# thethomasboyer/PhenDiff

Hardware: AMD Instinct MI355X
Metric: img2img images/sec (50-step DDIM invert+denoise, 256x256) (higher is better)
Workload: dtype bf16; 1 GPU; configs[2]: 256x256 pipeline_conditional_ddim invert->class-swap->denoise, 50+50 DDIM steps, super_small UNet (random init, seed 0), 3k_steps_clipping_rescaling, 32 images/GPU/step sharded over 1 GPU(s), no collectives; batch_per_gpu=32, global_batch=32, inference_steps=50, image_size=256, hipgraph=True, concurrent_trajectories=1

## Files before the change

phendiff_amd/csrc/attn_d8.hip:

```cpp
#include <stdlib.h>
#include <type_traits>
#include "pd_common.h"

namespace pd {

constexpr int KT = 256;
static_assert(KT == 256, "knmax is read as one f32x4 (KT / 64 slices)");

typedef uint32_t u32x4 __attribute__((ext_vector_type(4)));

__device__ __forceinline__ float row16_max(float x) {
#define PD_DPP_MAX(ctrl) x = fmaxf(x, __int_as_float(__builtin_amdgcn_update_dpp(__float_as_int(x), __float_as_int(x), ctrl, 0xf, 0xf, false)))
  PD_DPP_MAX(0xB1);
  PD_DPP_MAX(0x4E);
  PD_DPP_MAX(0x141);
  PD_DPP_MAX(0x140);
#undef PD_DPP_MAX
  return x;
}

__device__ __forceinline__ unsigned short bits16(bf16_t v) { return v; }
__device__ __forceinline__ unsigned short bits16(half_t v) { return v.bits; }

template <typename T> struct AttnOps {
  static constexpr float RESCALE_THR = sizeof(T) == 2 && !std::is_same<T, bf16_t>::value ? 14.0f : 16.0f;
  static constexpr int VT_PITCH = (KT + 8) * 2;
  struct QF { s16x8 v; };
  static __device__ __forceinline__ QF load_q(const T* q, int h, float scale) {
    QF f; f.v = (s16x8)(0);
    if (h == 0) {
      s16x8 raw = *(const s16x8*)q;
      {
        float x[8];
        typename Elem<T>::Frag fr; fr.v = raw;
        Elem<T>::unpack(fr, x);
#pragma unroll
        for (int j = 0; j < 8; ++j) x[j] *= scale;
        f.v = Elem<T>::pack(x).v;
      }
    }
    return f;
  }
  static constexpr float M_C0 = std::is_same<T, bf16_t>::value ? 1.0f : 4096.0f;
  static constexpr bool M_IN_C = false;
  static __device__ __forceinline__ float set_m(QF& q, f32x16&, int h, float m) {
    const T hi = Elem<T>::from_f(-m * (1.0f / M_C0));
    const float r1 = fmaf(-M_C0, Elem<T>::to_f(hi), -m);
    const T mid = Elem<T>::from_f(r1);
    const float r2 = r1 - Elem<T>::to_f(mid);
    const T lo = Elem<T>::from_f(r2);
    if (h) { q.v[0] = (short)bits16(hi); q.v[1] = (short)bits16(mid); q.v[2] = (short)bits16(lo); }
    return -(fmaf(M_C0, Elem<T>::to_f(hi), Elem<T>::to_f(mid)) + Elem<T>::to_f(lo));
  }
  static __device__ __forceinline__ void split3(float x, T& hi, T& mid, T& lo) {
    hi = Elem<T>::from_f(x * (1.0f / M_C0));
    const float r1 = fmaf(-M_C0, Elem<T>::to_f(hi), x);
    mid = Elem<T>::from_f(r1);
    lo = Elem<T>::from_f(r1 - Elem<T>::to_f(mid));
  }
  static __device__ __forceinline__ void set_terms(QF& q, int h, float c) {
    T hi, mid, lo;
    split3(c, hi, mid, lo);
    if (h) { q.v[0] = (short)bits16(hi); q.v[1] = (short)bits16(mid); q.v[2] = (short)bits16(lo); }
  }
  static __device__ __forceinline__ void set_ones(QF& q, int h) {
    if (h) { q.v[0] = (short)bits16(Elem<T>::from_f(M_C0)); q.v[1] = (short)bits16(Elem<T>::from_f(1.0f)); q.v[2] = q.v[1]; }
  }
  static __device__ __forceinline__ void store_terms(unsigned char* row16, float c) {
    T t[8];
    split3(c, t[0], t[1], t[2]);
#pragma unroll
    for (int i = 3; i < 8; ++i) t[i] = Elem<T>::from_f(0.0f);
    *(s16x8*)row16 = *(const s16x8*)t;
  }
  static __device__ __forceinline__ void init_const_slot(unsigned char* slot) {
    T c[8];
#pragma unroll
    for (int i = 0; i < 8; ++i) c[i] = Elem<T>::from_f(i == 0 ? M_C0 : i < 3 ? 1.0f : 0.0f);
    *(s16x8*)slot = *(const s16x8*)c;
  }
  static __device__ __forceinline__ float q_norm2(const QF& q) {
    float x[8], t = 0.f;
    typename Elem<T>::Frag fr; fr.v = q.v;
    Elem<T>::unpack(fr, x);
#pragma unroll
    for (int j = 0; j < 8; ++j) t += x[j] * x[j];
    return t;
  }
  static __device__ __forceinline__ float dot(const QF& x, const QF& y) {
    float a[8], b[8], t = 0.f;
    typename Elem<T>::Frag fa, fb; fa.v = x.v; fb.v = y.v;
    Elem<T>::unpack(fa, a); Elem<T>::unpack(fb, b);
#pragma unroll
    for (int j = 0; j < 8; ++j) t += a[j] * b[j];
    return t;
  }
  static __device__ __forceinline__ float k_norm2(const typename Elem<T>::Frag& k) {
    const u32x4 w = __builtin_bit_cast(u32x4, k.v);
    float n2 = 0.f;
    if constexpr (std::is_same<T, bf16_t>::value) {
      typedef __bf16 bf2 __attribute__((ext_vector_type(2)));
#pragma unroll
      for (int j = 0; j < 4; ++j) {
        const uint32_t wj = w[j];
        const bf2 pr = __builtin_bit_cast(bf2, wj);
        n2 = __builtin_amdgcn_fdot2_f32_bf16(pr, pr, n2, false);
      }
    } else {
      float x[8];
      Elem<T>::unpack(k, x);
#pragma unroll
      for (int j = 0; j < 8; ++j) n2 += x[j] * x[j];
    }
    return n2;
  }
  static __device__ __forceinline__ void store_vt(unsigned char* vl, int vp, const typename Elem<T>::Frag& v) {
#pragma unroll
    for (int d = 0; d < 8; ++d) *(unsigned short*)(vl + d * VT_PITCH + vp * 2) = (unsigned short)v.v[d];
  }
  static constexpr int KROW = 16;
  static constexpr int KSTEP = 32 * KROW;
  static __device__ __forceinline__ int kaddr(int r, int h) { return h ? KT * KROW : r * KROW; }
  static __device__ __forceinline__ int kstep(int h) { return h ? 0 : KSTEP; }
  struct KF { s16x8 v; };
  struct VF { u32x4 v[2]; };
  static __device__ __forceinline__ KF load_k(const unsigned char* ka) { KF f; f.v = *(const s16x8*)ka; return f; }
  static __device__ __forceinline__ f32x16 qk(const KF& a, const QF& q, const f32x16& c) {
    return Elem<T>::mma16(a.v, q.v, c);
  }
  static __device__ __forceinline__ VF load_v(const unsigned char* vrow, int key0) {
    VF f;
    f.v[0] = *(const u32x4*)(vrow + key0 * 2);
    f.v[1] = *(const u32x4*)(vrow + (key0 + 16) * 2);
    return f;
  }
  static __device__ __forceinline__ int vpos(int t) { return t ^ ((((t >> 2) ^ (t >> 3)) & 1) * 12); }
  static __device__ __forceinline__ int vlane_off(int h) { return h * 16; }
  static __device__ __forceinline__ uint32_t pack_p(float lo, float hi) {
    if constexpr (std::is_same<T, bf16_t>::value) return __builtin_amdgcn_perm(__float_as_uint(hi), __float_as_uint(lo), 0x07060302u);
    else return Pack16<T>::pack(lo, hi);
  }
  static __device__ __forceinline__ f32x16 pv(const VF& a, const f32x16& p, f32x16 o) {
#pragma unroll
    for (int s = 0; s < 2; ++s) {
      uint32_t bw[4];
#pragma unroll
      for (int j = 0; j < 4; ++j) bw[j] = pack_p(p[8 * s + 2 * j], p[8 * s + 2 * j + 1]);
      u32x4 bv = {bw[0], bw[1], bw[2], bw[3]};
      o = Elem<T>::mma16(__builtin_bit_cast(s16x8, a.v[s]), __builtin_bit_cast(s16x8, bv), o);
    }
    return o;
  }
};

template <> struct AttnOps<float> {
  static constexpr float RESCALE_THR = 16.0f;
  static constexpr int VT_PITCH = (KT + 4) * 4;
  struct QF { f32x4 v; };
  static __device__ __forceinline__ QF load_q(const float* q, int h, float scale) {
    QF f; f.v = *(const f32x4*)(q + 4 * h);
    f.v *= scale;
    return f;
  }
  static constexpr bool M_IN_C = true;
  static __device__ __forceinline__ float set_m(QF&, f32x16& negm, int, float m) { negm = (f32x16)(-m); return m; }
  static __device__ __forceinline__ void init_const_slot(unsigned char*) {}
  static __device__ __forceinline__ float q_norm2(const QF& q) {
    return q.v[0] * q.v[0] + q.v[1] * q.v[1] + q.v[2] * q.v[2] + q.v[3] * q.v[3];
  }
  static __device__ __forceinline__ float dot(const QF& x, const QF& y) {
    return x.v[0] * y.v[0] + x.v[1] * y.v[1] + x.v[2] * y.v[2] + x.v[3] * y.v[3];
  }
  static __device__ __forceinline__ float k_norm2(const Elem<float>::Frag& k) {
    float n2 = 0.f;
#pragma unroll
    for (int j = 0; j < 4; ++j) n2 += k.lo[j] * k.lo[j] + k.hi[j] * k.hi[j];
    return n2;
  }
  static __device__ __forceinline__ void store_vt(unsigned char* vl, int vp, const Elem<float>::Frag& v) {
#pragma unroll
    for (int d = 0; d < 4; ++d) { *(float*)(vl + d * VT_PITCH + vp * 4) = v.lo[d]; *(float*)(vl + (4 + d) * VT_PITCH + vp * 4) = v.hi[d]; }
  }
  static constexpr int KROW = 32;
  static constexpr int KSTEP = 32 * KROW;
  static __device__ __forceinline__ int kaddr(int r, int h) { return r * KROW + h * 16; }
  static __device__ __forceinline__ int kstep(int) { return KSTEP; }
  static __device__ __forceinline__ int vpos(int t) { return t; }
  static __device__ __forceinline__ int vlane_off(int h) { return h * 16; }
  struct KF { f32x4 v; };
  struct VF { f32x4 v[4]; };
  static __device__ __forceinline__ KF load_k(const unsigned char* ka) { KF f; f.v = *(const f32x4*)ka; return f; }
  static __device__ __forceinline__ f32x16 qk(const KF& a, const QF& q, f32x16 c) {
#pragma unroll
    for (int i = 0; i < 4; ++i) c = __builtin_amdgcn_mfma_f32_32x32x2f32(a.v[i], q.v[i], c, 0, 0, 0);
    return c;
  }
  static __device__ __forceinline__ VF load_v(const unsigned char* vrow, int key0) {
    VF f;
#pragma unroll
    for (int g = 0; g < 4; ++g) f.v[g] = *(const f32x4*)(vrow + (key0 + 8 * g) * 4);
    return f;
  }
  static __device__ __forceinline__ f32x16 pv(const VF& a, const f32x16& p, f32x16 o) {
#pragma unroll
    for (int g = 0; g < 4; ++g)
#pragma unroll
      for (int i = 0; i < 4; ++i) o = __builtin_amdgcn_mfma_f32_32x32x2f32(a.v[g][i], p[4 * g + i], o, 0, 0, 0);
    return o;
  }
};

template <typename T, int QB, int WPB>
__global__ __launch_bounds__(WPB * 64) void attn_kernel(const pd_attn_args a) {
  constexpr int QPW = 32 * QB;
  constexpr int QPB = WPB * QPW;
  using E = Elem<T>;
  using Ops = AttnOps<T>;
  constexpr bool PIPE = sizeof(T) == 2 && QB == 1;
  constexpr int KROW = Ops::KROW;
  constexpr int VBYTES = 10 * Ops::VT_PITCH;
  __shared__ __attribute__((aligned(16))) unsigned char klds[2][KT * KROW + 16];
  __shared__ __attribute__((aligned(16))) unsigned char vlds[2][VBYTES];
  __shared__ __attribute__((aligned(16))) float knmax[2][KT / 64];

  const int tid = threadIdx.x, lane = tid & 63, wave = tid >> 6;
  const int r = lane & 31, h = lane >> 5;
  const int nqb = (a.N + QPB - 1) / QPB;
  const int total = nqb * a.heads * a.B;
  int item = blockIdx.x;
  if ((total & 7) == 0) item = (blockIdx.x & 7) * (total >> 3) + (blockIdx.x >> 3);
  const int qb = item % nqb;
  const int head = (item / nqb) % a.heads, b = item / (nqb * a.heads);
  const int N = a.N;
  const size_t bh = ((size_t)b * a.heads + head) * N;
  const T* qp = (const T*)a.q + bh * 8;
  const T* kp = (const T*)a.k + bh * 8;
  const T* vp = (const T*)a.v + bh * 8;

  const float qscale = 0.35355339059327373f * 1.4426950408889634f;
  constexpr float RESCALE_THR = Ops::RESCALE_THR;
  int query[QB];
  typename Ops::QF qf[QB];
  f32x16 o[QB], negm[QB];
  float qn[QB], m[QB];
  bool first[QB];
#pragma unroll
  for (int j = 0; j < QB; ++j) {
    query[j] = qb * QPB + (wave * QB + j) * 32 + r;
    qf[j] = Ops::load_q(qp + (size_t)min(query[j], N - 1) * 8, h, qscale);
    float t = Ops::q_norm2(qf[j]);
    t += __shfl_xor(t, 32);
    qn[j] = sqrtf(t) * 1.00001f + 1e-6f;
    o[j] = (f32x16)(0.f); negm[j] = (f32x16)(0.f); m[j] = 0.f; first[j] = true;
  }

#pragma unroll
  for (int b2 = 0; b2 < 2; ++b2) {
    if (tid == 0) { *(f32x4*)(klds[b2] + KT * KROW) = (f32x4)(0.f); Ops::init_const_slot(klds[b2] + KT * KROW); }
    if (tid < KT) { *(T*)(vlds[b2] + 8 * Ops::VT_PITCH + tid * E::BYTES) = E::from_f(1.0f); *(T*)(vlds[b2] + 9 * Ops::VT_PITCH + tid * E::BYTES) = E::from_f(0.0f); }
  }
  const int vrow_off = (r < 8 ? r : (r == 8 || r == 12) ? 8 : 9) * Ops::VT_PITCH + Ops::vlane_off(h);
  const int ka0 = Ops::kaddr(r, h), kst = Ops::kstep(h);

  const int st = tid & (KT - 1);
  const int my_parity = (WPB * 64 > KT) ? (tid / KT) : 0;
  auto mine = [&](int tile) { return (WPB * 64 > KT) ? ((tile & 1) == my_parity) : true; };
  typename E::Frag stk, stv;
  auto issue = [&](int k0) {
    if (!mine(k0 / KT)) return;
    const int key = k0 + st;
    if (key < N) { stk = E::load(kp + (size_t)key * 8); stv = E::load(vp + (size_t)key * 8); }
    else { stk = E::zero(); stv = E::zero(); }
  };
  auto commit = [&](int b2, int k0) {
    if (!mine(k0 / KT)) return;
    E::store(klds[b2] + st * KROW, stk);
    float n2 = row16_max(Ops::k_norm2(stk));
    n2 = fmaxf(n2, __shfl_xor(n2, 16));
    n2 = fmaxf(n2, __shfl_xor(n2, 32));
    if ((st & 63) == 0) knmax[b2][st >> 6] = sqrtf(n2) * 1.00002f;
    Ops::store_vt(vlds[b2], Ops::vpos(st), stv);
  };

  issue(0);
  commit(0, 0);
  if (KT < N) issue(KT);
  __syncthreads();
  for (int k0 = 0, cur = 0; k0 < N; k0 += KT, cur ^= 1) {
    const unsigned char* kl = klds[cur];
    const unsigned char* vrow = vlds[cur] + vrow_off;
    const f32x4 kn4 = *(const f32x4*)knmax[cur];
    const float kn8 = fmaxf(fmaxf(kn4[0], kn4[1]), fmaxf(kn4[2], kn4[3]));
    const bool full_tile = k0 + KT <= N;
    bool need = false;
#pragma unroll
    for (int j = 0; j < QB; ++j) need = need || first[j] || (qn[j] * kn8 - m[j] > RESCALE_THR);
    if (full_tile && !__builtin_amdgcn_ballot_w64(need)) {
      if constexpr (PIPE) {
        typename Ops::KF kfn = Ops::load_k(kl + ka0);
        typename Ops::VF vfn = Ops::load_v(vrow, 0);
        f32x16 sn = Ops::qk(kfn, qf[0], negm[0]);
        kfn = Ops::load_k(kl + ka0 + kst);
#pragma unroll
        for (int sub = 0; sub < KT / 32; ++sub) {
          const typename Ops::VF vf = vfn;
          f32x16 s = sn;
          if (sub + 1 < KT / 32) {
            sn = Ops::qk(kfn, qf[0], negm[0]);
            if (sub + 2 < KT / 32) kfn = Ops::load_k(kl + ka0 + (sub + 2) * kst);
            vfn = Ops::load_v(vrow, (sub + 1) * 32);
            __builtin_amdgcn_sched_barrier(0);
          }
#pragma unroll
          for (int i = 0; i < 16; ++i) s[i] = __builtin_amdgcn_exp2f(s[i]);
          o[0] = Ops::pv(vf, s, o[0]);
        }
      } else {
#pragma unroll
        for (int sub = 0; sub < KT / 32; ++sub) {
          const typename Ops::KF kf = Ops::load_k(kl + ka0 + sub * kst);
          const typename Ops::VF vf = Ops::load_v(vrow, sub * 32);
          f32x16 s[QB];
#pragma unroll
          for (int j = 0; j < QB; ++j) s[j] = Ops::qk(kf, qf[j], negm[j]);
#pragma unroll
          for (int j = 0; j < QB; ++j) {
#pragma unroll
            for (int i = 0; i < 16; ++i) s[j][i] = __builtin_amdgcn_exp2f(s[j][i]);
            o[j] = Ops::pv(vf, s[j], o[j]);
          }
        }
      }
    } else {
#pragma unroll 1
      for (int sub = 0; sub < KT / 32; ++sub) {
        const int kb = sub * 32;
        if (k0 + kb >= N) break;
        const typename Ops::KF kf = Ops::load_k(kl + ka0 + sub * kst);
        const typename Ops::VF vf = Ops::load_v(vrow, kb);
#pragma unroll
        for (int j = 0; j < QB; ++j) {
          f32x16 s = Ops::qk(kf, qf[j], negm[j]);
          if (k0 + kb + 32 > N) {
#pragma unroll
            for (int i = 0; i < 16; ++i) {
              const int key = k0 + kb + (i & 3) + 8 * (i >> 2) + 4 * h;
              if (key >= N) s[i] = -INFINITY;
            }
          }
          const float bound = qn[j] * knmax[cur][sub >> 1] - m[j];
          if (__builtin_amdgcn_ballot_w64(first[j] || bound > RESCALE_THR)) {
            float tmax = s[0];
#pragma unroll
            for (int i = 1; i < 16; ++i) tmax = fmaxf(tmax, s[i]);
            if (__builtin_amdgcn_ballot_w64(first[j] || tmax > RESCALE_THR)) {
              const float t2 = fmaxf(tmax, __shfl_xor(tmax, 32));
              const float m_new = Ops::set_m(qf[j], negm[j], h, m[j] + (first[j] ? t2 : fmaxf(t2, 0.f)));
              const float delta = m_new - m[j];
              const float sc = first[j] ? 1.f : __builtin_amdgcn_exp2f(-delta);
#pragma unroll
              for (int i = 0; i < 8; ++i) o[j][i] *= sc;
#pragma unroll
              for (int i = 0; i < 16; ++i) s[i] -= delta;
              m[j] = m_new;
              first[j] = false;
            }
          }
#pragma unroll
          for (int i = 0; i < 16; ++i) s[i] = __builtin_amdgcn_exp2f(s[i]);
          o[j] = Ops::pv(vf, s, o[j]);
        }
      }
    }
    if (k0 + KT < N) {
      commit(cur ^ 1, k0 + KT);
      if (k0 + 2 * KT < N) issue(k0 + 2 * KT);
    }
    __syncthreads();
  }

#pragma unroll
  for (int j = 0; j < QB; ++j) {
    if (query[j] < N) {
      const float inv = 1.0f / o[j][4];
      if (a.lse && h == 0) a.lse[bh + query[j]] = m[j] + __builtin_amdgcn_logf(o[j][4]);
      T* dst = (T*)a.out + ((size_t)b * N + query[j]) * (a.heads * 8) + head * 8 + 4 * h;
      store4(dst, o[j][0] * inv, o[j][1] * inv, o[j][2] * inv, o[j][3] * inv);
    }
  }
}


constexpr int ATTN_DMA_KT = 256;
template <typename T>
__global__ __launch_bounds__(512) void attn_glds_kernel(const pd_attn_args a) {
  static_assert(sizeof(T) == 2, "16-bit element types");
  using Ops = AttnOps<T>;
  constexpr int KT = ATTN_DMA_KT;
  constexpr int KROW = 16, TILE = KT * KROW;
  constexpr int ONES = TILE + 256;
  constexpr int K_OFF = 0, V_OFF = 2 * TILE, ONES_OFF = 4 * TILE, KCONST_OFF = 4 * TILE + ONES;
  __shared__ __attribute__((aligned(1024))) unsigned char lds[4 * TILE + ONES + 16];

  const int tid = threadIdx.x, lane = tid & 63, wave = tid >> 6;
  const int r = lane & 31, h = lane >> 5;
  const int nqb = (a.N + 255) / 256;
  const int total = nqb * a.heads * a.B;
  int item = blockIdx.x;
  if ((total & 7) == 0) item = (blockIdx.x & 7) * (total >> 3) + (blockIdx.x >> 3);
  const int qb = item % nqb;
  const int head = (item / nqb) % a.heads, b = item / (nqb * a.heads);
  const int N = a.N;
  const size_t bh = ((size_t)b * a.heads + head) * N;
  const T* qp = (const T*)a.q + bh * 8;

  const float qscale = 0.35355339059327373f * 1.4426950408889634f;
  constexpr float RESCALE_THR = Ops::RESCALE_THR;
  const int query = qb * 256 + wave * 32 + r;
  typename Ops::QF qf = Ops::load_q(qp + (size_t)min(query, N - 1) * 8, h, qscale);
  float qn = Ops::q_norm2(qf);
  qn += __shfl_xor(qn, 32);
  qn = sqrtf(qn) * 1.00001f + 1e-6f;
  const float kn = sqrtf(a.kmax2[b * a.heads + head]) * 1.00002f;
  float qk_bound = qn * kn;
  f32x16 o = (f32x16)(0.f), zero = (f32x16)(0.f);
  float m = 0.f;

  if (tid == 0) Ops::init_const_slot(lds + KCONST_OFF);
  for (int i16 = tid; i16 < ONES / 16; i16 += 512) {
    T one8[8];
#pragma unroll
    for (int i = 0; i < 8; ++i) one8[i] = Elem<T>::from_f(i == 0 ? 1.0f : 0.0f);
    *(s16x8*)(lds + ONES_OFF + i16 * 16) = *(const s16x8*)one8;
  }
  const int koff = h ? KCONST_OFF : K_OFF + r * KROW;
  const int kst = h ? 0 : 32 * KROW, kbuf = h ? 0 : TILE;
  const int tq = (lane & 15) >> 2, tp = lane & 3;
  const bool vrow = (lane & 16) == 0 && tp < 2;
  const int voff = vrow ? V_OFF + (4 * h + tq) * KROW + 8 * tp : ONES_OFF + (16 * h + 16) * 4 + ((lane & 16) ? 8 : 0);
  const int vbuf = vrow ? TILE : 0;
  auto load_v = [&](int base, int sub) {
    typedef short v4s __attribute__((ext_vector_type(4)));
    typedef __attribute__((address_space(3))) v4s* lp;
    typename Ops::VF f;
#pragma unroll
    for (int s2 = 0; s2 < 2; ++s2) {
      const v4s lo = __builtin_amdgcn_ds_read_tr16_b64_v4i16((lp)(lds + base + (32 * sub + 16 * s2) * KROW));
      const v4s hi = __builtin_amdgcn_ds_read_tr16_b64_v4i16((lp)(lds + base + (32 * sub + 16 * s2 + 8) * KROW));
      const s16x8 fr = {lo[0], lo[1], lo[2], lo[3], hi[0], hi[1], hi[2], hi[3]};
      f.v[s2] = __builtin_bit_cast(u32x4, fr);
    }
    return f;
  };

  const unsigned char* gsrc = (const unsigned char*)((const T*)(wave < 4 ? a.k : a.v) + bh * 8);
  const unsigned lds_base = (unsigned)(size_t)(__attribute__((address_space(3))) unsigned char*)lds;
  const unsigned sdst = __builtin_amdgcn_readfirstlane(lds_base + (wave < 4 ? K_OFF : V_OFF) + (wave & 3) * 1024);
  auto stage = [&](int b2, int k0) {
    #pragma unroll
    for (int pc = 0; pc < KT / 256; ++pc) {
      const int key = min(k0 + ((wave & 3) + 4 * pc) * 64 + lane, N - 1);
      const unsigned char* src = gsrc + (size_t)key * 16;
      const unsigned dst = sdst + b2 * TILE + pc * 4096;
      unsigned keep;
      asm volatile("s_mov_b32 %0, m0\n\ts_mov_b32 m0, %2\n\ts_nop 0\n\tglobal_load_lds_dwordx4 %1, off\n\ts_mov_b32 m0, %0"
                   : "=&s"(keep) : "v"(src), "s"(dst) : "memory");
    }
  };

  stage(0, 0);
  asm volatile("s_waitcnt vmcnt(0)" ::: "memory");
  __syncthreads();
  {
    const f32x16 s0 = Ops::qk(Ops::load_k(lds + koff), qf, zero);
    float tmax = s0[0];
#pragma unroll
    for (int i = 1; i < 16; ++i) tmax = fmaxf(tmax, s0[i]);
    tmax = fmaxf(tmax, __shfl_xor(tmax, 32));
    m = Ops::set_m(qf, zero, h, tmax);
    if (tmax > qk_bound) qk_bound = INFINITY;
  }
  for (int k0 = 0, cur = 0; k0 < N; k0 += KT, cur ^= 1) {
    if (k0 + KT < N) stage(cur ^ 1, k0 + KT);
    const int kl = koff + cur * kbuf;
    const int vb = voff + cur * vbuf;
    const bool full_tile = k0 + KT <= N;
    const bool need = qk_bound - m > RESCALE_THR;
    if (full_tile && !__builtin_amdgcn_ballot_w64(need)) {
      typename Ops::KF kfn = Ops::load_k(lds + kl);
      typename Ops::VF vfn = load_v(vb, 0);
      f32x16 sn = Ops::qk(kfn, qf, zero);
      kfn = Ops::load_k(lds + kl + kst);
#pragma unroll
      for (int sub = 0; sub < KT / 32; ++sub) {
        const typename Ops::VF vf = vfn;
        f32x16 s = sn;
        if (sub + 1 < KT / 32) {
          sn = Ops::qk(kfn, qf, zero);
          if (sub + 2 < KT / 32) kfn = Ops::load_k(lds + kl + (sub + 2) * kst);
          vfn = load_v(vb, sub + 1);
          __builtin_amdgcn_sched_barrier(0);
        }
#pragma unroll
        for (int i = 0; i < 16; ++i) s[i] = __builtin_amdgcn_exp2f(s[i]);
        o = Ops::pv(vf, s, o);
      }
    } else {
#pragma unroll 1
      for (int sub = 0; sub < KT / 32; ++sub) {
        const int kb = sub * 32;
        if (k0 + kb >= N) break;
        const typename Ops::KF kf = Ops::load_k(lds + kl + sub * kst);
        const typename Ops::VF vf = load_v(vb, sub);
        f32x16 s = Ops::qk(kf, qf, zero);
        if (k0 + kb + 32 > N) {
#pragma unroll
          for (int i = 0; i < 16; ++i) {
            const int key = k0 + kb + (i & 3) + 8 * (i >> 2) + 4 * h;
            if (key >= N) s[i] = -INFINITY;
          }
        }
        if (__builtin_amdgcn_ballot_w64(qk_bound - m > RESCALE_THR)) {
          float tmax = s[0];
#pragma unroll
          for (int i = 1; i < 16; ++i) tmax = fmaxf(tmax, s[i]);
          if (__builtin_amdgcn_ballot_w64(tmax > RESCALE_THR)) {
            const float t2 = fmaxf(tmax, __shfl_xor(tmax, 32));
            const float m_new = Ops::set_m(qf, zero, h, m + fmaxf(t2, 0.f));
            const float delta = m_new - m;
            const float sc = __builtin_amdgcn_exp2f(-delta);
#pragma unroll
            for (int i = 0; i < 8; ++i) o[i] *= sc;
#pragma unroll
            for (int i = 0; i < 16; ++i) s[i] -= delta;
            m = m_new;
          }
        }
#pragma unroll
        for (int i = 0; i < 16; ++i) s[i] = __builtin_amdgcn_exp2f(s[i]);
        o = Ops::pv(vf, s, o);
      }
    }
    asm volatile("s_waitcnt vmcnt(0)" ::: "memory");
    __syncthreads();
  }

  if (query < N) {
    const float inv = 1.0f / o[4];
    if (a.lse && h == 0) a.lse[bh + query] = m + __builtin_amdgcn_logf(o[4]);
    T* dst = (T*)a.out + ((size_t)b * N + query) * (a.heads * 8) + head * 8 + 4 * h;
    store4(dst, o[0] * inv, o[1] * inv, o[2] * inv, o[3] * inv);
  }
}

template <typename T>
__global__ __launch_bounds__(256) void attn_bwd_dq_kernel(const pd_attn_bwd_args a) {
  using E = Elem<T>;
  using Ops = AttnOps<T>;
  constexpr int KROW = Ops::KROW;
  __shared__ __attribute__((aligned(16))) unsigned char klds[2][KT * KROW + 16];
  __shared__ __attribute__((aligned(16))) unsigned char vlds[2][KT * KROW + 16];
  __shared__ __attribute__((aligned(16))) unsigned char ktlds[2][9 * Ops::VT_PITCH];

  const int tid = threadIdx.x, lane = tid & 63, wave = tid >> 6;
  const int r = lane & 31, h = lane >> 5;
  const int nqb = (a.N + 127) / 128;
  const int total = nqb * a.heads * a.B;
  int item = blockIdx.x;
  if ((total & 7) == 0) item = (blockIdx.x & 7) * (total >> 3) + (blockIdx.x >> 3);
  const int qb = item % nqb;
  const int head = (item / nqb) % a.heads, b = item / (nqb * a.heads);
  const int N = a.N, C = a.heads * 8;
  const size_t bh = ((size_t)b * a.heads + head) * N;
  const T* kp = (const T*)a.k + bh * 8;
  const T* vp = (const T*)a.v + bh * 8;
  const float qscale = 0.35355339059327373f * 1.4426950408889634f;

  const int query = qb * 128 + wave * 32 + r, qc = min(query, N - 1);
  const typename Ops::QF qf0 = Ops::load_q((const T*)a.q + (bh + qc) * 8, h, qscale);
  const typename Ops::QF dof0 = Ops::load_q((const T*)a.dout + ((size_t)b * N + qc) * C + head * 8, h, 1.0f);
  const typename Ops::QF of = Ops::load_q((const T*)a.o + ((size_t)b * N + qc) * C + head * 8, h, 1.0f);
  float delta = Ops::dot(dof0, of);
  delta += __shfl_xor(delta, 32);
  if (h == 0 && query < N) a.delta[bh + query] = delta;
  constexpr bool SLOTS = !Ops::M_IN_C;
  f32x16 negl = (f32x16)(0.f), negd = (f32x16)(0.f);
  typename Ops::QF qf = qf0, dof = dof0;
  if constexpr (SLOTS) { Ops::set_terms(qf, h, -a.lse[bh + qc]); Ops::set_terms(dof, h, -delta); }
  else { negl = (f32x16)(-a.lse[bh + qc]); negd = (f32x16)(-delta); }
  f32x16 dq = (f32x16)(0.f);

#pragma unroll
  for (int b2 = 0; b2 < 2; ++b2) {
    if (tid == 0) {
      *(f32x4*)(klds[b2] + KT * KROW) = (f32x4)(0.f); *(f32x4*)(vlds[b2] + KT * KROW) = (f32x4)(0.f);
      if constexpr (SLOTS) { Ops::init_const_slot(klds[b2] + KT * KROW); Ops::init_const_slot(vlds[b2] + KT * KROW); }
    }
    *(T*)(ktlds[b2] + 8 * Ops::VT_PITCH + tid * E::BYTES) = E::from_f(0.0f);
  }
  const int vrow_off = (r < 8 ? r : 8) * Ops::VT_PITCH + Ops::vlane_off(h);
  const int ka0 = Ops::kaddr(r, h), kst = Ops::kstep(h);

  typename E::Frag stk, stv;
  auto issue = [&](int k0) {
    const int key = k0 + tid;
    if (key < N) { stk = E::load(kp + (size_t)key * 8); stv = E::load(vp + (size_t)key * 8); }
    else { stk = E::zero(); stv = E::zero(); }
  };
  auto commit = [&](int b2) {
    E::store(klds[b2] + tid * KROW, stk);
    E::store(vlds[b2] + tid * KROW, stv);
    float kv[8];
    E::unpack(stk, kv);
    const int vp_ = Ops::vpos(tid);
#pragma unroll
    for (int d = 0; d < 8; ++d) *(T*)(ktlds[b2] + d * Ops::VT_PITCH + vp_ * E::BYTES) = E::from_f(kv[d]);
  };
  auto body = [&](const unsigned char* kl, const unsigned char* vl, const unsigned char* ktrow, int sub) {
    const typename Ops::KF kf = Ops::load_k(kl + ka0 + sub * kst);
    const typename Ops::KF vf = Ops::load_k(vl + ka0 + sub * kst);
    const typename Ops::VF ktf = Ops::load_v(ktrow, sub * 32);
    f32x16 s = Ops::qk(kf, qf, negl);
    const f32x16 dp = Ops::qk(vf, dof, negd);
#pragma unroll
    for (int i = 0; i < 16; ++i) s[i] = __builtin_amdgcn_exp2f(s[i]) * dp[i];
    dq = Ops::pv(ktf, s, dq);
  };

  issue(0);
  commit(0);
  if (KT < N) issue(KT);
  __syncthreads();
  for (int k0 = 0, cur = 0; k0 < N; k0 += KT, cur ^= 1) {
    const unsigned char* kl = klds[cur];
    const unsigned char* vl = vlds[cur];
    const unsigned char* ktrow = ktlds[cur] + vrow_off;
    if (k0 + KT <= N) {
#pragma unroll
      for (int sub = 0; sub < KT / 32; ++sub) body(kl, vl, ktrow, sub);
    } else {
#pragma unroll 1
      for (int sub = 0; sub < KT / 32 && k0 + sub * 32 < N; ++sub) body(kl, vl, ktrow, sub);
    }
    if (k0 + KT < N) {
      commit(cur ^ 1);
      if (k0 + 2 * KT < N) issue(k0 + 2 * KT);
    }
    __syncthreads();
  }
  if (query < N) {
    const float sc = 0.35355339059327373f;
    T* dst = (T*)a.dqkv + ((size_t)b * N + query) * (3 * C) + head * 8 + 4 * h;
    store4(dst, dq[0] * sc, dq[1] * sc, dq[2] * sc, dq[3] * sc);
  }
}

template <typename T>
__global__ __launch_bounds__(256) void attn_bwd_dkv_kernel(const pd_attn_bwd_args a) {
  using E = Elem<T>;
  using Ops = AttnOps<T>;
  constexpr int KROW = Ops::KROW;
  constexpr int QT = sizeof(T) == 4 ? 128 : 256;
  constexpr bool SLOTS = !Ops::M_IN_C;
  constexpr int ROWS = SLOTS ? 2 * QT * KROW : QT * KROW + 16;
  __shared__ __attribute__((aligned(16))) unsigned char qlds[2][ROWS];
  __shared__ __attribute__((aligned(16))) unsigned char dolds[2][ROWS];
  __shared__ __attribute__((aligned(16))) unsigned char qtlds[2][9 * Ops::VT_PITCH];
  __shared__ __attribute__((aligned(16))) unsigned char dotlds[2][9 * Ops::VT_PITCH];
  __shared__ __attribute__((aligned(16))) float nl[2][SLOTS ? 4 : QT], nd[2][SLOTS ? 4 : QT];

  const int tid = threadIdx.x, lane = tid & 63, wave = tid >> 6;
  const int r = lane & 31, h = lane >> 5;
  const int nkb = (a.N + 127) / 128;
  const int total = nkb * a.heads * a.B;
  int item = blockIdx.x;
  if ((total & 7) == 0) item = (blockIdx.x & 7) * (total >> 3) + (blockIdx.x >> 3);
  const int kb = item % nkb;
  const int head = (item / nkb) % a.heads, b = item / (nkb * a.heads);
  const int N = a.N, C = a.heads * 8;
  const size_t bh = ((size_t)b * a.heads + head) * N;
  const T* qp = (const T*)a.q + bh * 8;
  const T* dop = (const T*)a.dout + (size_t)b * N * C + head * 8;
  const float qscale = 0.35355339059327373f * 1.4426950408889634f;

  const int key = kb * 128 + wave * 32 + r, kc = min(key, N - 1);
  typename Ops::QF kfr = Ops::load_q((const T*)a.k + (bh + kc) * 8, h, 1.0f);
  typename Ops::QF vfr = Ops::load_q((const T*)a.v + (bh + kc) * 8, h, 1.0f);
  if constexpr (SLOTS) { Ops::set_ones(kfr, h); Ops::set_ones(vfr, h); }
  f32x16 dk = (f32x16)(0.f), dv = (f32x16)(0.f);

#pragma unroll
  for (int b2 = 0; b2 < 2; ++b2) {
    if constexpr (!SLOTS) {
      if (tid == 0) { *(f32x4*)(qlds[b2] + QT * KROW) = (f32x4)(0.f); *(f32x4*)(dolds[b2] + QT * KROW) = (f32x4)(0.f); }
    }
    if (tid < QT) {
      *(T*)(qtlds[b2] + 8 * Ops::VT_PITCH + tid * E::BYTES) = E::from_f(0.0f);
      *(T*)(dotlds[b2] + 8 * Ops::VT_PITCH + tid * E::BYTES) = E::from_f(0.0f);
    }
  }
  const int vrow_off = (r < 8 ? r : 8) * Ops::VT_PITCH + Ops::vlane_off(h);
  const int ka0 = SLOTS ? (h ? QT * KROW + r * KROW : r * KROW) : Ops::kaddr(r, h);
  const int kst = SLOTS ? 32 * KROW : Ops::kstep(h);

  typename E::Frag stq, stdo;
  float stl = 0.f, std_ = 0.f;
  auto issue = [&](int q0) {
    const int query = q0 + tid;
    if (tid < QT && query < N) {
      stq = E::load(qp + (size_t)query * 8); stdo = E::load(dop + (size_t)query * C);
      stl = -a.lse[bh + query]; std_ = -a.delta[bh + query];
    } else { stq = E::zero(); stdo = E::zero(); stl = 0.f; std_ = 0.f; }
  };
  auto commit = [&](int b2) {
    if (tid < QT) {
      float qv[8], dv_[8];
      E::unpack(stq, qv);
#pragma unroll
      for (int d = 0; d < 8; ++d) qv[d] *= qscale;
      const typename E::Frag qs = E::pack(qv);
      E::store(qlds[b2] + tid * KROW, qs);
      E::store(dolds[b2] + tid * KROW, stdo);
      E::unpack(qs, qv);
      E::unpack(stdo, dv_);
      const int vp_ = Ops::vpos(tid);
#pragma unroll
      for (int d = 0; d < 8; ++d) {
        *(T*)(qtlds[b2] + d * Ops::VT_PITCH + vp_ * E::BYTES) = E::from_f(qv[d]);
        *(T*)(dotlds[b2] + d * Ops::VT_PITCH + vp_ * E::BYTES) = E::from_f(dv_[d]);
      }
      if constexpr (SLOTS) {
        Ops::store_terms(qlds[b2] + (QT + tid) * KROW, stl);
        Ops::store_terms(dolds[b2] + (QT + tid) * KROW, std_);
      } else { nl[b2][tid] = stl; nd[b2][tid] = std_; }
    }
  };
  auto body = [&](int cur, int sub) {
    const typename Ops::KF qa = Ops::load_k(qlds[cur] + ka0 + sub * kst);
    const typename Ops::KF doa = Ops::load_k(dolds[cur] + ka0 + sub * kst);
    f32x16 cl = (f32x16)(0.f), cd = (f32x16)(0.f);
    if constexpr (!SLOTS) {
#pragma unroll
      for (int g = 0; g < 4; ++g) {
        const f32x4 l4 = *(const f32x4*)&nl[cur][sub * 32 + 8 * g + 4 * h];
        const f32x4 d4 = *(const f32x4*)&nd[cur][sub * 32 + 8 * g + 4 * h];
#pragma unroll
        for (int i = 0; i < 4; ++i) { cl[4 * g + i] = l4[i]; cd[4 * g + i] = d4[i]; }
      }
    }
    f32x16 p = Ops::qk(qa, kfr, cl);
    f32x16 ds = Ops::qk(doa, vfr, cd);
#pragma unroll
    for (int i = 0; i < 16; ++i) { p[i] = __builtin_amdgcn_exp2f(p[i]); ds[i] *= p[i]; }
    dv = Ops::pv(Ops::load_v(dotlds[cur] + vrow_off, sub * 32), p, dv);
    dk = Ops::pv(Ops::load_v(qtlds[cur] + vrow_off, sub * 32), ds, dk);
  };

  issue(0);
  commit(0);
  if (QT < N) issue(QT);
  __syncthreads();
  for (int q0 = 0, cur = 0; q0 < N; q0 += QT, cur ^= 1) {
    if (q0 + QT <= N) {
#pragma unroll
      for (int sub = 0; sub < QT / 32; ++sub) body(cur, sub);
    } else {
#pragma unroll 1
      for (int sub = 0; sub < QT / 32 && q0 + sub * 32 < N; ++sub) body(cur, sub);
    }
    if (q0 + QT < N) {
      commit(cur ^ 1);
      if (q0 + 2 * QT < N) issue(q0 + 2 * QT);
    }
    __syncthreads();
  }
  if (key < N) {
    const float ln2 = 0.6931471805599453f;
    T* dst = (T*)a.dqkv + ((size_t)b * N + key) * (3 * C) + head * 8 + 4 * h;
    store4(dst + C, dk[0] * ln2, dk[1] * ln2, dk[2] * ln2, dk[3] * ln2);
    store4(dst + 2 * C, dv[0], dv[1], dv[2], dv[3]);
  }
}


constexpr int FUSED_TR_PITCH = 72;
constexpr int FUSED_TR_IMG = 32 * FUSED_TR_PITCH;
template <typename T, int NSUB>
__global__ __launch_bounds__(512) void attn_bwd_fused_kernel(const pd_attn_bwd_args a, float* __restrict__ slab, int nkb) {
  static_assert(sizeof(T) == 2, "16-bit element types");
  using E = Elem<T>;
  using Ops = AttnOps<T>;
  constexpr int KROW = 16, QT = 256, KPB = 256 * NSUB;
  constexpr int ROWS = 2 * QT * KROW;
  constexpr int VTB = 9 * Ops::VT_PITCH;
  constexpr int Q_OFF = 0, DO_OFF = 2 * ROWS, QT_OFF = 4 * ROWS, DOT_OFF = 4 * ROWS + 2 * VTB, TR_OFF = 4 * ROWS + 4 * VTB,
                DQ_OFF = TR_OFF + 8 * 2 * FUSED_TR_IMG;
  extern __shared__ __attribute__((aligned(16))) unsigned char lds[];

  const int tid = threadIdx.x, lane = tid & 63, wave = tid >> 6;
  const int r = lane & 31, h = lane >> 5;
  const int total = nkb * a.heads * a.B;
  int item = blockIdx.x;
  if ((total & 7) == 0) item = (blockIdx.x & 7) * (total >> 3) + (blockIdx.x >> 3);
  const int kb = item % nkb;
  const int head = (item / nkb) % a.heads, b = item / (nkb * a.heads);
  const int N = a.N, C = a.heads * 8;
  const size_t bh = ((size_t)b * a.heads + head) * N;
  const T* qp = (const T*)a.q + bh * 8;
  const T* dop = (const T*)a.dout + (size_t)b * N * C + head * 8;
  const T* op = (const T*)a.o + (size_t)b * N * C + head * 8;
  const float qscale = 0.35355339059327373f * 1.4426950408889634f;

  typename Ops::QF kfr[NSUB], vfr[NSUB];
  s16x8 kt[NSUB][2];
  f32x16 dk[NSUB], dv[NSUB];
#pragma unroll
  for (int ks = 0; ks < NSUB; ++ks) {
    const int key0 = kb * KPB + (wave * NSUB + ks) * 32;
    const int key = key0 + r, kc = min(key, N - 1);
    kfr[ks] = Ops::load_q((const T*)a.k + (bh + kc) * 8, h, 1.0f);
    vfr[ks] = Ops::load_q((const T*)a.v + (bh + kc) * 8, h, 1.0f);
    Ops::set_ones(kfr[ks], h); Ops::set_ones(vfr[ks], h);
    dk[ks] = (f32x16)(0.f); dv[ks] = (f32x16)(0.f);
#pragma unroll
    for (int s2 = 0; s2 < 2; ++s2) {
      s16x8 f = (s16x8)(0);
      if (r < 8) {
#pragma unroll
        for (int j = 0; j < 8; ++j) {
          const int kk = key0 + 16 * s2 + 8 * h + j;
          if (kk < N) f[j] = (short)bits16(((const T*)a.k)[(bh + kk) * 8 + r]);
        }
      }
      kt[ks][s2] = f;
    }
  }

#pragma unroll
  for (int b2 = 0; b2 < 2; ++b2) {
    if (tid < QT) {
      *(T*)(lds + QT_OFF + b2 * VTB + 8 * Ops::VT_PITCH + tid * E::BYTES) = E::from_f(0.0f);
      *(T*)(lds + DOT_OFF + b2 * VTB + 8 * Ops::VT_PITCH + tid * E::BYTES) = E::from_f(0.0f);
    }
  }
  const int vrow_off = (r < 8 ? r : 8) * Ops::VT_PITCH + Ops::vlane_off(h);
  const int ka0 = h ? QT * KROW + r * KROW : r * KROW;
  constexpr int kst = 32 * KROW;
  unsigned char* const trw = lds + TR_OFF + wave * (2 * FUSED_TR_IMG);
  const int tr_rd = ((lane & 15) >> 2) * FUSED_TR_PITCH + (16 * ((lane >> 4) & 1) + 4 * (lane & 3)) * 2 + 8 * h * FUSED_TR_PITCH;
  const int tr_wr = r * FUSED_TR_PITCH + 8 * h;
  float* const dq_mine = (float*)(lds + DQ_OFF) + wave * (QT * 8);

  typename E::Frag stq, stdo, sto;
  float stl = 0.f;
  auto issue = [&](int q0) {
    const int query = q0 + tid;
    if (tid < QT && query < N) {
      stq = E::load(qp + (size_t)query * 8); stdo = E::load(dop + (size_t)query * C); sto = E::load(op + (size_t)query * C);
      stl = -a.lse[bh + query];
    } else { stq = E::zero(); stdo = E::zero(); sto = E::zero(); stl = 0.f; }
  };
  auto commit = [&](int b2, int q0) {
    if (tid < QT) {
      float qv[8], dv_[8], ov[8];
      E::unpack(stq, qv);
#pragma unroll
      for (int d = 0; d < 8; ++d) qv[d] *= qscale;
      const typename E::Frag qs = E::pack(qv);
      E::store(lds + Q_OFF + b2 * ROWS + tid * KROW, qs);
      E::store(lds + DO_OFF + b2 * ROWS + tid * KROW, stdo);
      E::unpack(qs, qv);
      E::unpack(stdo, dv_);
      E::unpack(sto, ov);
      float delta = 0.f;
#pragma unroll
      for (int d = 0; d < 8; ++d) delta += dv_[d] * ov[d];
      const int vp_ = Ops::vpos(tid);
#pragma unroll
      for (int d = 0; d < 8; ++d) {
        *(T*)(lds + QT_OFF + b2 * VTB + d * Ops::VT_PITCH + vp_ * E::BYTES) = E::from_f(qv[d]);
        *(T*)(lds + DOT_OFF + b2 * VTB + d * Ops::VT_PITCH + vp_ * E::BYTES) = E::from_f(dv_[d]);
      }
      Ops::store_terms(lds + Q_OFF + b2 * ROWS + (QT + tid) * KROW, stl);
      Ops::store_terms(lds + DO_OFF + b2 * ROWS + (QT + tid) * KROW, -delta);
      if (kb == 0 && q0 + tid < N) a.delta[bh + q0 + tid] = delta;
    }
  };
  typedef short v4s __attribute__((ext_vector_type(4)));
  typedef __attribute__((address_space(3))) v4s* lp;
  typedef uint32_t u32x2 __attribute__((ext_vector_type(2)));
  auto step = [&](int cur, int sub, f32x16& dq) {
    constexpr int ATTN_BWD_IGLP = 3;
    __builtin_amdgcn_iglp_opt(ATTN_BWD_IGLP);
    const typename Ops::KF qa = Ops::load_k(lds + Q_OFF + cur * ROWS + ka0 + sub * kst);
    const typename Ops::KF doa = Ops::load_k(lds + DO_OFF + cur * ROWS + ka0 + sub * kst);
    const typename Ops::VF dotf = Ops::load_v(lds + DOT_OFF + cur * VTB + vrow_off, sub * 32);
    const typename Ops::VF qtf = Ops::load_v(lds + QT_OFF + cur * VTB + vrow_off, sub * 32);
    const f32x16 zero = (f32x16)(0.f);
    f32x16 p[NSUB], ds[NSUB];
#pragma unroll
    for (int ks = 0; ks < NSUB; ++ks) {
      p[ks] = Ops::qk(qa, kfr[ks], zero);
      ds[ks] = Ops::qk(doa, vfr[ks], zero);
    }
    uint32_t bw[NSUB][2][4];
#pragma unroll
    for (int ks = 0; ks < NSUB; ++ks) {
#pragma unroll
      for (int i = 0; i < 16; ++i) { p[ks][i] = __builtin_amdgcn_exp2f(p[ks][i]); ds[ks][i] *= p[ks][i]; }
#pragma unroll
      for (int s2 = 0; s2 < 2; ++s2)
#pragma unroll
        for (int j = 0; j < 4; ++j) bw[ks][s2][j] = Ops::pack_p(ds[ks][8 * s2 + 2 * j], ds[ks][8 * s2 + 2 * j + 1]);
#pragma unroll
      for (int g = 0; g < 4; ++g) {
        const u32x2 w2 = {bw[ks][g >> 1][(g & 1) * 2], bw[ks][g >> 1][(g & 1) * 2 + 1]};
        *(u32x2*)(trw + ks * FUSED_TR_IMG + tr_wr + 16 * g) = w2;
      }
    }
#pragma unroll
    for (int ks = 0; ks < NSUB; ++ks) {
      dv[ks] = Ops::pv(dotf, p[ks], dv[ks]);
#pragma unroll
      for (int s2 = 0; s2 < 2; ++s2) {
        const u32x4 bv = {bw[ks][s2][0], bw[ks][s2][1], bw[ks][s2][2], bw[ks][s2][3]};
        dk[ks] = E::mma16(__builtin_bit_cast(s16x8, qtf.v[s2]), __builtin_bit_cast(s16x8, bv), dk[ks]);
      }
#pragma unroll
      for (int s2 = 0; s2 < 2; ++s2) {
        const v4s lo = __builtin_amdgcn_ds_read_tr16_b64_v4i16((lp)(trw + ks * FUSED_TR_IMG + tr_rd + (16 * s2) * FUSED_TR_PITCH));
        const v4s hi = __builtin_amdgcn_ds_read_tr16_b64_v4i16((lp)(trw + ks * FUSED_TR_IMG + tr_rd + (16 * s2 + 4) * FUSED_TR_PITCH));
        const s16x8 bt = {lo[0], lo[1], lo[2], lo[3], hi[0], hi[1], hi[2], hi[3]};
        dq = E::mma16(kt[ks][s2], bt, dq);
      }
    }
  };

  issue(0);
  commit(0, 0);
  if (QT < N) issue(QT);
  __syncthreads();
  for (int q0 = 0, cur = 0; q0 < N; q0 += QT, cur ^= 1) {
    const int nsub = min(8, (N - q0 + 31) / 32);
#pragma unroll 1
    for (int sub = 0; sub < nsub; ++sub) {
      f32x16 dq = (f32x16)(0.f);
      step(cur, sub, dq);
      *(f32x4*)(dq_mine + (sub * 32 + r) * 8 + 4 * h) = (f32x4){dq[0], dq[1], dq[2], dq[3]};
    }
    __syncthreads();
    {
      const int query = q0 + (tid >> 1), half = tid & 1;
      if (query < N) {
        f32x4 v = (f32x4)(0.f);
#pragma unroll
        for (int w = 0; w < 8; ++w) v += *(const f32x4*)((const float*)(lds + DQ_OFF) + w * (QT * 8) + tid * 4);
        if (nkb == 1) {
          const float sc = 0.35355339059327373f;
          store4((T*)a.dqkv + ((size_t)b * N + query) * (3 * C) + head * 8 + 4 * half, v[0] * sc, v[1] * sc, v[2] * sc, v[3] * sc);
        } else {
          *(f32x4*)(slab + (((size_t)kb * a.B * a.heads + (size_t)b * a.heads + head) * N + query) * 8 + 4 * half) = v;
        }
      }
    }
    if (q0 + QT < N) {
      commit(cur ^ 1, q0 + QT);
      if (q0 + 2 * QT < N) issue(q0 + 2 * QT);
    }
    __syncthreads();
  }
  const float ln2 = 0.6931471805599453f;
#pragma unroll
  for (int ks = 0; ks < NSUB; ++ks) {
    const int key = kb * KPB + (wave * NSUB + ks) * 32 + r;
    if (key < N) {
      T* dst = (T*)a.dqkv + ((size_t)b * N + key) * (3 * C) + head * 8 + 4 * h;
      store4(dst + C, dk[ks][0] * ln2, dk[ks][1] * ln2, dk[ks][2] * ln2, dk[ks][3] * ln2);
      store4(dst + 2 * C, dv[ks][0], dv[ks][1], dv[ks][2], dv[ks][3]);
    }
  }
}

template <typename T>
__global__ __launch_bounds__(256) void attn_dq_reduce_kernel(const float* __restrict__ slab, int nkb, int B, int heads, int N, T* __restrict__ dqkv) {
  const size_t i = (size_t)blockIdx.x * 256 + threadIdx.x;
  if (i >= (size_t)B * heads * N) return;
  const int n = (int)(i % N), head = (int)((i / N) % heads), b = (int)(i / ((size_t)N * heads));
  const size_t per = (size_t)B * heads * N * 8;
  f32x4 lo = (f32x4)(0.f), hi = (f32x4)(0.f);
  for (int k = 0; k < nkb; ++k) {
    lo += *(const f32x4*)(slab + k * per + i * 8);
    hi += *(const f32x4*)(slab + k * per + i * 8 + 4);
  }
  const float sc = 0.35355339059327373f;
  T* dst = dqkv + ((size_t)b * N + n) * (3 * heads * 8) + head * 8;
  store4(dst, lo[0] * sc, lo[1] * sc, lo[2] * sc, lo[3] * sc);
  store4(dst + 4, hi[0] * sc, hi[1] * sc, hi[2] * sc, hi[3] * sc);
}

}

extern "C" int pd_attn_d8(const pd_attn_args* a, void* stream) {
  using namespace pd;
  PD_CHECK(a != nullptr, PD_ERR_ARG, "pd_attn_d8: null args");
  PD_CHECK(a->B > 0 && a->heads > 0 && a->N > 0, PD_ERR_SHAPE, "pd_attn_d8: bad shape");
  PD_CHECK(a->q && a->k && a->v && a->out, PD_ERR_ARG, "pd_attn_d8: null pointer");
  const bool wpb4_only = diag_env("PD_ATTN_WPB4", 0) != 0;
  const bool wide = !wpb4_only && a->N >= 1024 && (long long)(a->N / 256) * a->heads * a->B >= 1024;
  const int qpb = wide ? 256 : 128;
  PD_CHECK((long long)((a->N + qpb - 1) / qpb) * a->heads * a->B < (1ll << 31), PD_ERR_SHAPE, "pd_attn_d8: grid too large");
  dim3 grid(((a->N + qpb - 1) / qpb) * a->heads * a->B);
  hipStream_t st = (hipStream_t)stream;
  static const int lds_pad = getenv("PD_ATTN_LDS_PAD") ? atoi(getenv("PD_ATTN_LDS_PAD")) : 0;
  if (lds_pad > 0 && a->dtype == PD_BF16 && wide) {
    static LdsAttr attr_a, attr_b;
    (void)ensure_lds(attr_a, attn_kernel<bf16_t, 1, 8>, lds_pad);
    (void)ensure_lds(attr_b, attn_glds_kernel<bf16_t>, lds_pad);
    if (a->kmax2) hipLaunchKernelGGL((attn_glds_kernel<bf16_t>), grid, dim3(512), lds_pad, st, *a);
    else hipLaunchKernelGGL((attn_kernel<bf16_t, 1, 8>), grid, dim3(512), lds_pad, st, *a);
    PD_LAUNCH_CHECK();
    return PD_OK;
  }
  const bool no_glds = diag_env("PD_ATTN_NO_GLDS", 0) != 0;
  if (a->kmax2 && wide && !no_glds && a->dtype != PD_F32) {
    if (a->dtype == PD_BF16) hipLaunchKernelGGL((attn_glds_kernel<bf16_t>), grid, dim3(512), 0, st, *a);
    else if (a->dtype == PD_F16) {
      hipLaunchKernelGGL((attn_glds_kernel<half_t>), grid, dim3(512), 0, st, *a);
    } else { set_error("pd_attn_d8: bad dtype"); return PD_ERR_ARG; }
    PD_LAUNCH_CHECK();
    return PD_OK;
  }
  if (a->dtype == PD_F32) {
    hipLaunchKernelGGL((attn_kernel<float, 1, 4>), dim3(((a->N + 127) / 128) * a->heads * a->B), dim3(256), 0, st, *a);
  } else if (a->dtype == PD_BF16) {
    if (wide) hipLaunchKernelGGL((attn_kernel<bf16_t, 1, 8>), grid, dim3(512), 0, st, *a);
    else hipLaunchKernelGGL((attn_kernel<bf16_t, 1, 4>), grid, dim3(256), 0, st, *a);
  } else if (a->dtype == PD_F16) {
    if (wide) hipLaunchKernelGGL((attn_kernel<half_t, 1, 8>), grid, dim3(512), 0, st, *a);
    else hipLaunchKernelGGL((attn_kernel<half_t, 1, 4>), grid, dim3(256), 0, st, *a);
  } else { set_error("pd_attn_d8: bad dtype"); return PD_ERR_ARG; }
  PD_LAUNCH_CHECK();
  return PD_OK;
}


static constexpr int FUSED_KPB = 512;
extern "C" size_t pd_attn_d8_bwd_workspace(const pd_attn_bwd_args* a) {
  if (!a || a->dtype == PD_F32 || a->B < 1 || a->heads < 1 || a->N < FUSED_KPB) return 0;
  const size_t nkb = ((size_t)a->N + FUSED_KPB - 1) / FUSED_KPB;
  return nkb * (size_t)a->B * a->heads * a->N * 8 * sizeof(float);
}

template <typename T>
static int launch_attn_bwd_fused(const pd_attn_bwd_args* a, hipStream_t st) {
  using namespace pd;
  constexpr int LDS = 4 * (2 * 256 * 16) + 4 * (9 * AttnOps<T>::VT_PITCH) + 8 * 2 * FUSED_TR_IMG + 8 * 256 * 8 * 4;
  auto kern = attn_bwd_fused_kernel<T, 2>;
  static LdsAttr attr;
  if (!ensure_lds(attr, kern, LDS)) {
    set_error("pd_attn_d8_bwd: cannot reserve %d bytes of LDS", LDS);
    return PD_ERR_LAUNCH;
  }
  const int nkb = (a->N + FUSED_KPB - 1) / FUSED_KPB;
  PD_CHECK((long long)nkb * a->heads * a->B < (1ll << 31), PD_ERR_SHAPE, "pd_attn_d8_bwd: grid too large");
  hipLaunchKernelGGL(kern, dim3((unsigned)(nkb * a->heads * a->B)), dim3(512), LDS, st, *a, a->slab, nkb);
  PD_LAUNCH_CHECK();
  if (nkb > 1) {
    const size_t rows = (size_t)a->B * a->heads * a->N;
    hipLaunchKernelGGL(attn_dq_reduce_kernel<T>, dim3((unsigned)((rows + 255) / 256)), dim3(256), 0, st, (const float*)a->slab, nkb, a->B, a->heads, a->N,
                       (T*)a->dqkv);
    PD_LAUNCH_CHECK();
  }
  return PD_OK;
}

extern "C" int pd_attn_d8_bwd(const pd_attn_bwd_args* a, void* stream) {
  using namespace pd;
  PD_CHECK(a != nullptr, PD_ERR_ARG, "pd_attn_d8_bwd: null args");
  PD_CHECK(a->B > 0 && a->heads > 0 && a->N > 0, PD_ERR_SHAPE, "pd_attn_d8_bwd: bad shape");
  PD_CHECK(a->q && a->k && a->v && a->o && a->dout && a->lse && a->delta && a->dqkv, PD_ERR_ARG, "pd_attn_d8_bwd: null pointer");
  if (a->slab != nullptr && diag_env("PD_ATTN_BWD_FUSED", 1) != 0) {
    const size_t need = pd_attn_d8_bwd_workspace(a);
    if (need > 0 && a->slab_bytes >= need && (a->dtype == PD_BF16 || a->dtype == PD_F16)) {
      const int rc = a->dtype == PD_BF16 ? launch_attn_bwd_fused<bf16_t>(a, (hipStream_t)stream) : launch_attn_bwd_fused<half_t>(a, (hipStream_t)stream);
      if (rc != PD_ERR_LAUNCH) return rc;
    }
  }
  PD_CHECK((long long)((a->N + 127) / 128) * a->heads * a->B < (1ll << 31), PD_ERR_SHAPE, "pd_attn_d8_bwd: grid too large");
  const dim3 grid(((a->N + 127) / 128) * a->heads * a->B);
  hipStream_t st = (hipStream_t)stream;
  if (a->dtype == PD_F32) {
    hipLaunchKernelGGL(attn_bwd_dq_kernel<float>, grid, dim3(256), 0, st, *a);
    hipLaunchKernelGGL(attn_bwd_dkv_kernel<float>, grid, dim3(256), 0, st, *a);
  } else if (a->dtype == PD_BF16) {
    hipLaunchKernelGGL(attn_bwd_dq_kernel<bf16_t>, grid, dim3(256), 0, st, *a);
    hipLaunchKernelGGL(attn_bwd_dkv_kernel<bf16_t>, grid, dim3(256), 0, st, *a);
  } else if (a->dtype == PD_F16) {
    hipLaunchKernelGGL(attn_bwd_dq_kernel<half_t>, grid, dim3(256), 0, st, *a);
    hipLaunchKernelGGL(attn_bwd_dkv_kernel<half_t>, grid, dim3(256), 0, st, *a);
  } else { set_error("pd_attn_d8_bwd: bad dtype"); return PD_ERR_ARG; }
  PD_LAUNCH_CHECK();
  return PD_OK;
}
```

Baseline: 15.52 images/s.

## Hand-schedule exp/pack in bf16 attention fast path and split tile loops

For the bf16 attention kernel, the fast-tile inner loop now uses inline asm that interleaves v_exp_f32 for the next subtile's first scores with the v_perm packing of the current probabilities, so the transcendental unit overlaps with the packing and MFMA work. The constant-K slot is widened to a full tile so both half-waves use the same strided addressing. The per-tile fast/exact branch is replaced by three loops (exact prefix, fast middle, exact tail), which takes the ballot check out of the steady state. The cost is more LDS for the constant slot and fragile asm scheduling. Once the fast loop is entered the rescale check is never re-evaluated, which may alter numerical behaviour if the bound changes mid-sequence.

```diff
diff --git a/phendiff_amd/csrc/attn_d8.hip b/phendiff_amd/csrc/attn_d8.hip
--- a/phendiff_amd/csrc/attn_d8.hip
+++ b/phendiff_amd/csrc/attn_d8.hip
@@ -139,6 +139,27 @@
   static __device__ __forceinline__ uint32_t pack_p(float lo, float hi) {
     if constexpr (std::is_same<T, bf16_t>::value) return __builtin_amdgcn_perm(__float_as_uint(hi), __float_as_uint(lo), 0x07060302u);
     else return Pack16<T>::pack(lo, hi);
+  }
+  template <bool TAIL>
+  static __device__ __forceinline__ u32x4 pack4(float p0, float p1, float p2, float p3, float p4, float p5, float p6, float p7,
+                                                float& e0, float& e1, float& e2) {
+    static_assert(std::is_same<T, bf16_t>::value, "the truncating pack is the bf16 engine's");
+    uint32_t b0, b1, b2, b3;
+    float r0 = 0.f, r1 = 0.f, r2 = 0.f;
+#define PD_PACKS "v_perm_b32 %[b0], %[p1], %[p0], %[sel]\n\tv_perm_b32 %[b1], %[p3], %[p2], %[sel]\n\t" \
+                 "v_perm_b32 %[b2], %[p5], %[p4], %[sel]\n\tv_perm_b32 %[b3], %[p7], %[p6], %[sel]\n\t"
+    if constexpr (!TAIL) {
+      asm("v_exp_f32 %[r0], %[e0]\n\t" PD_PACKS "v_exp_f32 %[r1], %[e1]\n\tv_exp_f32 %[r2], %[e2]"
+          : [b0] "=&v"(b0), [b1] "=&v"(b1), [b2] "=&v"(b2), [b3] "=&v"(b3), [r0] "=&v"(r0), [r1] "=&v"(r1), [r2] "=&v"(r2)
+          : [p0] "v"(p0), [p1] "v"(p1), [p2] "v"(p2), [p3] "v"(p3), [p4] "v"(p4), [p5] "v"(p5), [p6] "v"(p6), [p7] "v"(p7), [e0] "v"(e0), [e1] "v"(e1), [e2] "v"(e2),
+            [sel] "s"(0x07060302u));
+      e0 = r0; e1 = r1; e2 = r2;
+    } else {
+      asm("s_nop 0\n\t" PD_PACKS "s_nop 1" : [b0] "=&v"(b0), [b1] "=&v"(b1), [b2] "=&v"(b2), [b3] "=&v"(b3)
+          : [p0] "v"(p0), [p1] "v"(p1), [p2] "v"(p2), [p3] "v"(p3), [p4] "v"(p4), [p5] "v"(p5), [p6] "v"(p6), [p7] "v"(p7), [sel] "s"(0x07060302u));
+    }
+#undef PD_PACKS
+    return u32x4{b0, b1, b2, b3};
   }
   static __device__ __forceinline__ f32x16 pv(const VF& a, const f32x16& p, f32x16 o) {
 #pragma unroll
@@ -400,7 +421,10 @@
   constexpr int KROW = 16, TILE = KT * KROW;
   constexpr int ONES = TILE + 256;
   constexpr int K_OFF = 0, V_OFF = 2 * TILE, ONES_OFF = 4 * TILE, KCONST_OFF = 4 * TILE + ONES;
-  __shared__ __attribute__((aligned(1024))) unsigned char lds[4 * TILE + ONES + 16];
+  constexpr bool BF = std::is_same<T, bf16_t>::value;
+  constexpr bool HAND = BF, KC = BF, LOOPS = BF;
+  constexpr int KCONST_BYTES = KC ? TILE : 16;
+  __shared__ __attribute__((aligned(1024))) unsigned char lds[4 * TILE + ONES + KCONST_BYTES];
 
   const int tid = threadIdx.x, lane = tid & 63, wave = tid >> 6;
   const int r = lane & 31, h = lane >> 5;
@@ -426,15 +450,15 @@
   f32x16 o = (f32x16)(0.f), zero = (f32x16)(0.f);
   float m = 0.f;
 
-  if (tid == 0) Ops::init_const_slot(lds + KCONST_OFF);
+  if (KC ? tid < KT : tid == 0) Ops::init_const_slot(lds + KCONST_OFF + (KC ? tid * KROW : 0));
   for (int i16 = tid; i16 < ONES / 16; i16 += 512) {
     T one8[8];
 #pragma unroll
     for (int i = 0; i < 8; ++i) one8[i] = Elem<T>::from_f(i == 0 ? 1.0f : 0.0f);
     *(s16x8*)(lds + ONES_OFF + i16 * 16) = *(const s16x8*)one8;
   }
-  const int koff = h ? KCONST_OFF : K_OFF + r * KROW;
-  const int kst = h ? 0 : 32 * KROW, kbuf = h ? 0 : TILE;
+  const int koff = (h ? KCONST_OFF : K_OFF) + ((KC || !h) ? r * KROW : 0);
+  const int kst = (KC || !h) ? 32 * KROW : 0, kbuf = h ? 0 : TILE;
   const int tq = (lane & 15) >> 2, tp = lane & 3;
   const bool vrow = (lane & 16) == 0 && tp < 2;
   const int voff = vrow ? V_OFF + (4 * h + tq) * KROW + 8 * tp : ONES_OFF + (16 * h + 16) * 4 + ((lane & 16) ? 8 : 0);
@@ -480,17 +504,18 @@
     m = Ops::set_m(qf, zero, h, tmax);
     if (tmax > qk_bound) qk_bound = INFINITY;
   }
-  for (int k0 = 0, cur = 0; k0 < N; k0 += KT, cur ^= 1) {
-    if (k0 + KT < N) stage(cur ^ 1, k0 + KT);
+  auto fast_tile = [&](int cur) {
     const int kl = koff + cur * kbuf;
     const int vb = voff + cur * vbuf;
-    const bool full_tile = k0 + KT <= N;
-    const bool need = qk_bound - m > RESCALE_THR;
-    if (full_tile && !__builtin_amdgcn_ballot_w64(need)) {
+    {
       typename Ops::KF kfn = Ops::load_k(lds + kl);
       typename Ops::VF vfn = load_v(vb, 0);
       f32x16 sn = Ops::qk(kfn, qf, zero);
       kfn = Ops::load_k(lds + kl + kst);
+      if constexpr (HAND) {
+#pragma unroll
+        for (int i = 0; i < 3; ++i) sn[i] = __builtin_amdgcn_exp2f(sn[i]);
+      }
 #pragma unroll
       for (int sub = 0; sub < KT / 32; ++sub) {
         const typename Ops::VF vf = vfn;
@@ -501,11 +526,38 @@
           vfn = load_v(vb, sub + 1);
           __builtin_amdgcn_sched_barrier(0);
         }
-#pragma unroll
-        for (int i = 0; i < 16; ++i) s[i] = __builtin_amdgcn_exp2f(s[i]);
-        o = Ops::pv(vf, s, o);
-      }
-    } else {
+        if constexpr (HAND) {
+          float e[16];
+#pragma unroll
+          for (int i = 0; i < 16; ++i) e[i] = s[i];
+#pragma unroll
+          for (int i = 3; i < 8; ++i) e[i] = __builtin_amdgcn_exp2f(e[i]);
+          const u32x4 b0 = Ops::template pack4<false>(e[0], e[1], e[2], e[3], e[4], e[5], e[6], e[7], e[8], e[9], e[10]);
+          o = Elem<T>::mma16(__builtin_bit_cast(s16x8, vf.v[0]), __builtin_bit_cast(s16x8, b0), o);
+#pragma unroll
+          for (int i = 11; i < 16; ++i) e[i] = __builtin_amdgcn_exp2f(e[i]);
+          u32x4 b1;
+          if (sub + 1 < KT / 32) {
+            float n0 = sn[0], n1 = sn[1], n2 = sn[2];
+            b1 = Ops::template pack4<false>(e[8], e[9], e[10], e[11], e[12], e[13], e[14], e[15], n0, n1, n2);
+            sn[0] = n0; sn[1] = n1; sn[2] = n2;
+          } else {
+            float n0 = 0.f, n1 = 0.f, n2 = 0.f;
+            b1 = Ops::template pack4<true>(e[8], e[9], e[10], e[11], e[12], e[13], e[14], e[15], n0, n1, n2);
+          }
+          o = Elem<T>::mma16(__builtin_bit_cast(s16x8, vf.v[1]), __builtin_bit_cast(s16x8, b1), o);
+        } else {
+#pragma unroll
+          for (int i = 0; i < 16; ++i) s[i] = __builtin_amdgcn_exp2f(s[i]);
+          o = Ops::pv(vf, s, o);
+        }
+      }
+    }
+  };
+  auto exact_tile = [&](int k0, int cur) {
+    const int kl = koff + cur * kbuf;
+    const int vb = voff + cur * vbuf;
+    {
 #pragma unroll 1
       for (int sub = 0; sub < KT / 32; ++sub) {
         const int kb = sub * 32;
@@ -541,8 +593,27 @@
         o = Ops::pv(vf, s, o);
       }
     }
+  };
+  auto begin_tile = [&](int k0, int cur) {
+    if (k0 + KT < N) stage(cur ^ 1, k0 + KT);
+  };
+  auto end_tile = [&]() {
     asm volatile("s_waitcnt vmcnt(0)" ::: "memory");
     __syncthreads();
+  };
+  auto fast_ok = [&](int k0) { return k0 + KT <= N && !__builtin_amdgcn_ballot_w64(qk_bound - m > RESCALE_THR); };
+  if constexpr (LOOPS) {
+    int k0 = 0, cur = 0;
+    for (; k0 < N && !fast_ok(k0); k0 += KT, cur ^= 1) { begin_tile(k0, cur); exact_tile(k0, cur); end_tile(); }
+    for (; k0 + KT <= N; k0 += KT, cur ^= 1) { begin_tile(k0, cur); fast_tile(cur); end_tile(); }
+    for (; k0 < N; k0 += KT, cur ^= 1) { begin_tile(k0, cur); exact_tile(k0, cur); end_tile(); }
+  } else {
+    for (int k0 = 0, cur = 0; k0 < N; k0 += KT, cur ^= 1) {
+      begin_tile(k0, cur);
+      if (fast_ok(k0)) fast_tile(cur);
+      else exact_tile(k0, cur);
+      end_tile();
+    }
   }
 
   if (query < N) {
```

After: 15.74 images/s (median of 6 runs). 1.01x the previous value.
